# idonahum/photoVerse

Measured on AMD Instinct MI355X. Metric: denoising steps/sec at 512x512 bs=16, 50-step loop (2 UNet fwd + CFG + DPM-Solver++ step per step), higher is better.
Workload: dtype f16; 1 GPU; configs[1] shape timed over 96 steps instead of 50: SD-v1.5 UNet + PhotoVerse processors, 96-step loop, bs=16/GPU, 512x512 (64x64 latents), P=1, guidance 7.5, fp16; per_gpu_batch=16, global_batch=16, latent=64, parallelism=dp1 (batch-sharded, 1 all_gather), hip_graph=True, graph_branches=2

## Files before the change

### photoverse_amd/csrc/pv_rowgemm.hip

```cpp
#include "pv_common.h"
#include <stdlib.h>

namespace {

constexpr int RG_K = 320;
constexpr int RG_CHUNK = 160;
constexpr int RG_TILE = RG_CHUNK * 128;
constexpr int RG_SLOTS = 4;
constexpr int RG_SMEM = RG_SLOTS * RG_TILE;

struct pv_rowgemm_params_dev : pv_row_gemm_params {
    uint32_t w_bytes;
};

template <int N>
__device__ __forceinline__ void rg_wait_vmcnt() {
    static_assert(N >= 0 && N < 64, "vmcnt is a 6-bit field");
    asm volatile("s_waitcnt vmcnt(%0)" ::"n"(N) : "memory");
}

template <bool GEGLU>
__global__ __launch_bounds__(256, 2) void row_gemm_kernel(const pv_rowgemm_params_dev p) {
    constexpr int C = RG_K;
    constexpr int KK = C / 32;
    constexpr int KT = C / 64;
    constexpr int NFC = RG_CHUNK / 16;
    typedef unsigned uint4_t __attribute__((ext_vector_type(4)));
    typedef unsigned uint2_t __attribute__((ext_vector_type(2)));
    extern __shared__ __attribute__((aligned(16))) char smem[];

    const int lane = pv_lane_id(), wave = pv_wave_id();
    const int fr = lane & 15, g = lane >> 4;
    const int m0 = (int)blockIdx.x * 128;
    const int rows_here = min(128, p.M - m0);
    const int n_chunks = p.N / RG_CHUNK;
    const int NT = n_chunks * KT;

    const __amdgpu_buffer_rsrc_t rw = __builtin_amdgcn_make_buffer_rsrc(const_cast<void*>(p.w), 0, (int)p.w_bytes, 0x00020000);
    const __amdgpu_buffer_rsrc_t rx = __builtin_amdgcn_make_buffer_rsrc(const_cast<half_t*>(reinterpret_cast<const half_t*>(p.x)) + (size_t)m0 * p.ld_x, 0,
                                                                        rows_here * p.ld_x * 2, 0x00020000);
    const int ld_o = p.ld_out;
    const __amdgpu_buffer_rsrc_t ro = __builtin_amdgcn_make_buffer_rsrc(reinterpret_cast<half_t*>(p.out) + (size_t)m0 * ld_o, 0, rows_here * ld_o * 2, 0x00020000);

    const int lrow = lane >> 3;
    const unsigned w_lane_off = (unsigned)lrow * (unsigned)(C * 2) + (unsigned)(((lane & 7) ^ lrow) << 4);
    const unsigned piece_off = w_lane_off + (unsigned)(wave * 8) * (unsigned)(C * 2);
    auto issue_stage = [&](int t) {
        const int nc = t / KT, kt = t - nc * KT;
        char* dst = smem + (t & (RG_SLOTS - 1)) * RG_TILE;
        const int soff = nc * RG_CHUNK * (C * 2) + kt * 128;
#pragma unroll
        for (int i = 0; i < 5; ++i)
            __builtin_amdgcn_raw_ptr_buffer_load_lds(rw, PV_LDS_PTR(dst + (wave + 4 * i) * 1024), 16, (int)piece_off, soff + i * 32 * (C * 2), 0, 0);
    };
    auto wg_barrier = [&]() {
        asm volatile("s_waitcnt lgkmcnt(0)" ::: "memory");
        __builtin_amdgcn_s_barrier();
        asm volatile("" ::: "memory");
    };

    half8_t xf[KK][2];
    int mrow[2];
#pragma unroll
    for (int qi = 0; qi < 2; ++qi) {
        mrow[qi] = wave * 32 + qi * 16 + fr;
        const int off = mrow[qi] * p.ld_x * 2 + g * 16;
#pragma unroll
        for (int kk = 0; kk < KK; ++kk) xf[kk][qi] = __builtin_bit_cast(half8_t, __builtin_amdgcn_raw_buffer_load_b128(rx, off, kk * 64, 0));
    }
    issue_stage(0);
    issue_stage(1);
    if (p.x_norm) {
        const float* tab = p.x_norm + (size_t)(m0 / p.rows_per_image) * 2 * C + g * 8;
#pragma unroll
        for (int kk = 0; kk < KK; ++kk) {
            const float4_t s0 = *reinterpret_cast<const float4_t*>(tab + kk * 32), s1 = *reinterpret_cast<const float4_t*>(tab + kk * 32 + 4);
            const float4_t h0 = *reinterpret_cast<const float4_t*>(tab + C + kk * 32), h1 = *reinterpret_cast<const float4_t*>(tab + C + kk * 32 + 4);
#pragma unroll
            for (int qi = 0; qi < 2; ++qi)
#pragma unroll
                for (int j = 0; j < 8; ++j) xf[kk][qi][j] = (half_t)((float)xf[kk][qi][j] * (j < 4 ? s0[j & 3] : s1[j & 3]) + (j < 4 ? h0[j & 3] : h1[j & 3]));
        }
    }
    if (p.ln) {
        typedef _Float16 h2_t __attribute__((ext_vector_type(2)));
        const h2_t ones = h2_t{(half_t)1.0f, (half_t)1.0f};
#pragma unroll
        for (int qi = 0; qi < 2; ++qi) {
            float sum = 0.f;
#pragma unroll
            for (int kk = 0; kk < KK; ++kk)
#pragma unroll
                for (int j = 0; j < 4; ++j) sum = __builtin_amdgcn_fdot2(h2_t{xf[kk][qi][2 * j], xf[kk][qi][2 * j + 1]}, ones, sum, false);
            const float mean = pv_quad_sum(sum) * (1.0f / (float)C);
            const half_t mh = (half_t)mean;
            const h2_t nm = h2_t{(half_t)(-mh), (half_t)(-mh)};
            float sq = 0.f;
#pragma unroll
            for (int kk = 0; kk < KK; ++kk)
#pragma unroll
                for (int j = 0; j < 4; ++j) {
                    const h2_t d = h2_t{xf[kk][qi][2 * j], xf[kk][qi][2 * j + 1]} + nm;
                    sq = __builtin_amdgcn_fdot2(d, d, sq, false);
                }
            const float dm = mean - (float)mh;
            const float var = pv_quad_sum(sq) * (1.0f / (float)C) - dm * dm;
            const float rstd = rsqrtf(fmaxf(var, 0.f) + p.ln_eps);
            const float nmr = -mean * rstd;
#pragma unroll
            for (int kk = 0; kk < KK; ++kk)
#pragma unroll
                for (int j = 0; j < 8; ++j) xf[kk][qi][j] = (half_t)fmaf((float)xf[kk][qi][j], rstd, nmr);
        }
    }
    rg_wait_vmcnt<0>();

    const int ring_lane[2] = {fr * 128 + ((g ^ (fr & 7)) << 4), fr * 128 + (((4 + g) ^ (fr & 7)) << 4)};
    const int pcol = (g & 1) ? 16 + (g - 1) * 4 : g * 4;
    constexpr int OUT_PER_CHUNK = GEGLU ? RG_CHUNK / 2 : RG_CHUNK;
    constexpr int STORES = GEGLU ? 6 : 10;

    float4_t acc[NFC][2];
    for (int it = 0; it < n_chunks / 2; ++it) {
        const int t0 = it * (2 * KT);
#pragma unroll
        for (int j = 0; j < 2 * KT; ++j) {
            const int t = t0 + j;
            const int kt = j % KT;
            const int nc = 2 * it + j / KT;
            if ((j & 1) == 0) {
                const bool stores_since = (j == 6) || (j == 0 && it > 0);
                if (t >= 2) {
                    if (stores_since) rg_wait_vmcnt<STORES>(); else rg_wait_vmcnt<0>();
                }
                wg_barrier();
                if (t + 2 < NT) issue_stage(t + 2);
                if (t + 3 < NT) issue_stage(t + 3);
            }
            if (kt == 0) {
#pragma unroll
                for (int i = 0; i < NFC; ++i)
                    acc[i][0] = acc[i][1] = p.bias ? *reinterpret_cast<const float4_t*>(p.bias + nc * RG_CHUNK + i * 16 + g * 4) : float4_t{0.f, 0.f, 0.f, 0.f};
            }
            const char* slot = smem + (t & (RG_SLOTS - 1)) * RG_TILE;
#pragma unroll
            for (int ks = 0; ks < 2; ++ks) {
                const char* base = slot + ring_lane[ks];
#pragma unroll
                for (int i = 0; i < NFC; ++i) {
                    const half8_t a = *reinterpret_cast<const half8_t*>(base + i * 2048);
#pragma unroll
                    for (int qi = 0; qi < 2; ++qi) acc[i][qi] = __builtin_amdgcn_mfma_f32_16x16x32_f16(a, xf[2 * kt + ks][qi], acc[i][qi], 0, 0, 0);
                }
            }
            if (kt == KT - 1) {
                const int ocol0 = nc * OUT_PER_CHUNK;
#pragma unroll
                for (int qi = 0; qi < 2; ++qi) {
                    const int ooff = mrow[qi] * ld_o * 2 + ocol0 * 2;
                    unsigned pk[GEGLU ? NFC / 2 : NFC][2];
                    if (GEGLU) {
#pragma unroll
                        for (int q = 0; q < NFC / 2; ++q) {
                            const float4_t v = acc[2 * q][qi], gt = acc[2 * q + 1][qi];
                            pk[q][0] = __builtin_bit_cast(unsigned, half2_t{(half_t)(v[0] * pv_gelu_erf(gt[0])), (half_t)(v[1] * pv_gelu_erf(gt[1]))});
                            pk[q][1] = __builtin_bit_cast(unsigned, half2_t{(half_t)(v[2] * pv_gelu_erf(gt[2])), (half_t)(v[3] * pv_gelu_erf(gt[3]))});
                        }
                    } else {
#pragma unroll
                        for (int i = 0; i < NFC; ++i) {
                            const float4_t v = acc[i][qi];
                            pk[i][0] = __builtin_bit_cast(unsigned, half2_t{(half_t)v[0], (half_t)v[1]});
                            pk[i][1] = __builtin_bit_cast(unsigned, half2_t{(half_t)v[2], (half_t)v[3]});
                        }
                    }
                    constexpr int NOUT = GEGLU ? NFC / 2 : NFC;
#pragma unroll
                    for (int q = 0; q < NOUT / 2; ++q) {
                        const auto v0 = __builtin_amdgcn_permlane16_swap(pk[2 * q][0], pk[2 * q + 1][0], false, false);
                        const auto v1 = __builtin_amdgcn_permlane16_swap(pk[2 * q][1], pk[2 * q + 1][1], false, false);
                        const unsigned sa0 = v0[0], sb0 = v0[1], sa1 = v1[0], sb1 = v1[1];
                        __builtin_amdgcn_raw_buffer_store_b128(uint4_t{sa0, sa1, sb0, sb1}, ro, ooff + pcol * 2 + q * 64, 0, 0);
                        asm volatile("s_nop 1" ::: "memory");
                    }
                    if (NOUT & 1)
                        __builtin_amdgcn_raw_buffer_store_b64(uint2_t{pk[NOUT - 1][0], pk[NOUT - 1][1]}, ro, ooff + g * 8 + (NOUT - 1) * 32, 0, 0);
                }
                __builtin_amdgcn_sched_barrier(0);
            }
        }
    }
}

}

extern "C" int pv_row_gemm(const pv_row_gemm_params* pp, void* stream) {
    pv_rowgemm_params_dev p;
    static_cast<pv_row_gemm_params&>(p) = *pp;
    if (!p.x || !p.w || !p.out || p.M <= 0 || p.K != RG_K || p.N <= 0 || (p.N % (2 * RG_CHUNK)) || (p.ld_x % 8) || (p.ld_out % 8) || p.ld_x < RG_K ||
        p.ld_out < (p.geglu ? p.N / 2 : p.N) || (p.x_norm && (p.ln || p.rows_per_image <= 0 || (p.rows_per_image % 128) || (p.M % p.rows_per_image))))
        return (int)hipErrorInvalidValue;
    if ((size_t)p.N * RG_K * 2 >= (1ull << 31)) return (int)hipErrorInvalidValue;
    p.w_bytes = (uint32_t)p.N * RG_K * 2;
    static bool attr_set_dev[64][2] = {};
    int dev_id = 0;
    (void)hipGetDevice(&dev_id);
    bool& attr_set = attr_set_dev[dev_id & 63][p.geglu ? 1 : 0];
    auto kern = p.geglu ? row_gemm_kernel<true> : row_gemm_kernel<false>;
    if (!attr_set) {
        hipError_t e = hipFuncSetAttribute(reinterpret_cast<const void*>(kern), hipFuncAttributeMaxDynamicSharedMemorySize, RG_SMEM);
        if (e != hipSuccess) return (int)e;
        attr_set = true;
    }
    hipLaunchKernelGGL(kern, dim3((unsigned)((p.M + 127) / 128)), dim3(256), RG_SMEM, (hipStream_t)stream, p);
    return PV_CHECK_LAUNCH();
}
```

### photoverse_amd/csrc/pv_convbig.hip

```cpp
#include "pv_gemm_dev.h"

#ifndef PV_PATCH_ABLATE
#define PV_PATCH_ABLATE 0
#endif
#ifdef PV_CONVBIG_STAMPS
__device__ unsigned long long pv_convbig_stamps[3 * 8 * 8];
extern "C" int pv_convbig_read_stamps(unsigned long long* out) { return (int)hipMemcpyFromSymbol(out, HIP_SYMBOL(pv_convbig_stamps), sizeof(pv_convbig_stamps)); }
#define CB_DECL unsigned long long cb_acc[4] = {0, 0, 0, 0}, cb_t = __builtin_amdgcn_s_memtime(), cb_u, cb_r0 = __builtin_amdgcn_s_memrealtime(), cb_c0 = cb_t; int cb_n = 0;
#define CB_MARK(i) do { cb_u = __builtin_amdgcn_s_memtime(); cb_acc[i] += cb_u - cb_t; cb_t = cb_u; } while (0)
#define CB_COUNT() (++cb_n)
#define CB_DUMP() do { const int slot_ = blockIdx.x == 0 ? 0 : blockIdx.x == 50 ? 1 : blockIdx.x == 100 ? 2 : -1; \
        if (slot_ >= 0 && lane == 0) { unsigned long long* o_ = pv_convbig_stamps + (slot_ * 8 + wave) * 8; \
            o_[0] = cb_acc[0]; o_[1] = cb_acc[1]; o_[2] = cb_acc[2]; o_[3] = cb_acc[3]; o_[4] = cb_t - cb_c0; o_[5] = __builtin_amdgcn_s_memrealtime() - cb_r0; o_[6] = cb_n; } } while (0)
#else
#define CB_DECL
#define CB_MARK(i)
#define CB_COUNT()
#define CB_DUMP()
#endif

namespace {

constexpr int BK = 32;
constexpr int ROW_BYTES = BK * 2;
// ... 18 lines not shown
    static constexpr int SMEM_NORM_BYTES = SMEM_PATCH_BYTES + NORM_TABLE_BYTES;
};

__device__ __forceinline__ float epi_act(float x, int act) {
    if (act == PV_ACT_SILU) return pv_silu(x);
    if (act == PV_ACT_QUICK_GELU) return pv_quick_gelu(x);
    if (act == PV_ACT_LEAKY_RELU) return x > 0.f ? x : 0.01f * x;
    return x;
}

__device__ __forceinline__ int swz(int rq) { return (0x78 >> (2 * rq)) & 3; }

template <int N>
__device__ __forceinline__ void wait_vmcnt() {
    asm volatile("s_waitcnt vmcnt(%0)" ::"n"(N) : "memory");
}

__device__ __forceinline__ float row16_sum(float v) {
    v += __builtin_bit_cast(float, __builtin_amdgcn_update_dpp(0, __builtin_bit_cast(int, v), 0x128, 0xf, 0xf, false));
    v += __builtin_bit_cast(float, __builtin_amdgcn_update_dpp(0, __builtin_bit_cast(int, v), 0x124, 0xf, 0xf, false));
    v += __builtin_bit_cast(float, __builtin_amdgcn_update_dpp(0, __builtin_bit_cast(int, v), 0x122, 0xf, 0xf, false));
    v += __builtin_bit_cast(float, __builtin_amdgcn_update_dpp(0, __builtin_bit_cast(int, v), 0x121, 0xf, 0xf, false));
    return v;
}

template <int V>
struct IC { static constexpr int value = V; };

template <bool CS, bool UPS, int MI, int MODE, bool LN = false>
__global__ __launch_bounds__(512, 2) void big_tile_kernel(const pv_gemm_params_dev p, const int tiles_n, const int nblk) {
    constexpr int NF = MODE == 2 ? 4 : 5;
    constexpr bool PATCH = MODE >= 3, NORMA = MODE >= 5;
    constexpr bool IS_CONV = MODE == 0 || PATCH;
    constexpr int LOG2W = (MODE == 3 || MODE == 5) ? 6 : 5, PW = 1 << LOG2W, PR = 256 >> LOG2W, PS = PW + 2, NPIX = (PR + 2) * PS;
    constexpr int TAPS = IS_CONV ? 9 : 1;
    using Cfg = BigCfg<MI, NF>;
    static_assert(!PATCH || (MI == 8 && !UPS && !LN), "the patch modes are the plain 256-row conv");
    static_assert(NPIX <= Cfg::PATCH_PIECES * 16, "the patch fits its 32 pieces");
    constexpr int BM = Cfg::BM, BN = Cfg::BN, AP = Cfg::AP, BP = Cfg::BP, B_PIECES = Cfg::B_PIECES, A_BYTES = Cfg::A_BYTES, STAGE_BYTES = Cfg::STAGE_BYTES;
    constexpr int P_HI = AP + BP, P_LO = AP + Cfg::BP_LO;
    static_assert(!UPS || MODE == 0, "the upsampling gather belongs to the conv");
    static_assert(!LN || (MODE != 0 && !CS), "the LayerNorm fold exists for the Linear modes (their outputs feed attention / a Linear: no column statistics)");
    extern __shared__ __attribute__((aligned(16))) char smem[];
    const int lane = pv_lane_id();
    const int wave = pv_wave_id();
    const int bid = pv_xcd_remap((int)blockIdx.x, nblk);
    const int tile_m = bid / tiles_n, tile_n = bid - tile_m * tiles_n;
    const int m0 = tile_m * BM, n0 = tile_n * BN;
    const int cin = p.c0 + p.c1;
    const int K = TAPS * cin;
    const int nk64 = K / 64;
    const int nk_per = (nk64 + (int)gridDim.y - 1) / (int)gridDim.y;
    const int kb = (int)blockIdx.y * nk_per;
    const int ns = 2 * max(0, min(nk64, kb + nk_per) - kb);

    constexpr unsigned OOB = 0x80000000u;
    const int hw_out = p.hout * p.wout;
    const int prow = lane >> 2;
    float4_t acc[NF][MI];
#pragma unroll
    for (int ni = 0; ni < NF; ++ni)
#pragma unroll
        for (int mi = 0; mi < MI; ++mi) acc[ni][mi] = float4_t{0.f, 0.f, 0.f, 0.f};

    const int wm = wave >> 2, wn = wave & 3;
    const int fr = lane & 15, fq = lane >> 4;
    const int arow = wm * (MI * 16) + fr;
    const int brow = wn * (NF * 16) + fr;
    const int frag_off = fr * ROW_BYTES + ((fq ^ swz((fr >> 2) & 3)) << 4);

    half8_t wb[NF], xa[MI];
    float ln_s1[LN ? MI : 1], ln_s2[LN ? MI : 1];
#pragma unroll
    for (int mi = 0; mi < (LN ? MI : 1); ++mi) ln_s1[mi] = ln_s2[mi] = 0.f;
    auto seg_barrier = [&]() {
        __builtin_amdgcn_sched_barrier(0);
        __builtin_amdgcn_s_barrier();
        asm volatile("" ::: "memory");
        __builtin_amdgcn_sched_barrier(0);
    };
    if constexpr (!PATCH) {
        const int lane_cc2 = ((lane & 3) ^ swz((lane >> 4) & 3)) * 16;
        const __amdgpu_buffer_rsrc_t ra0 = __builtin_amdgcn_make_buffer_rsrc(const_cast<void*>(p.a0), 0, (int)p.a0_bytes, 0x00020000);
        const __amdgpu_buffer_rsrc_t ra1 = __builtin_amdgcn_make_buffer_rsrc(const_cast<void*>(p.a1 ? p.a1 : p.a0), 0, (int)p.a1_bytes, 0x00020000);
        const __amdgpu_buffer_rsrc_t rw = __builtin_amdgcn_make_buffer_rsrc(const_cast<void*>(p.w), 0, (int)p.w_bytes, 0x00020000);
        unsigned a_off0[AP], a_off1[AP], a_mask[AP];
#pragma unroll
        for (int i = 0; i < AP; ++i) {
            const int m = m0 + (wave + i * NW) * 16 + prow;
            const bool ok = m < p.M;
            if (MODE != 0) {
                a_off0[i] = ok ? (unsigned)m * (unsigned)(p.lda0 * 2) + lane_cc2 : OOB;
                a_off1[i] = a_mask[i] = 0;
                continue;
            }
            const int b = m / hw_out;
            const int rem = m - b * hw_out;
            const int y = rem / p.wout, x = rem - y * p.wout;
            const int hl = UPS ? 2 * p.hin : p.hin, wl = UPS ? 2 * p.win : p.win;
            unsigned mask = 0;
#pragma unroll
            for (int t = 0; t < 9; ++t) {
                const int iy = y + t / 3 - 1, ix = x + t % 3 - 1;
                mask |= (ok && iy >= 0 && iy < hl && ix >= 0 && ix < wl) ? 1u << t : 0u;
            }
            if (UPS) mask |= (unsigned)(y & 1) << 9 | (unsigned)(x & 1) << 10;
            a_mask[i] = mask;
            const unsigned pix = UPS ? (unsigned)((b * p.hin + (y >> 1)) * p.win + (x >> 1)) : (unsigned)((b * p.hin + y) * p.win + x);
            a_off0[i] = pix * (unsigned)(p.lda0 * 2) + lane_cc2;
            a_off1[i] = pix * (unsigned)(p.lda1 * 2) + lane_cc2;
        }
        unsigned w_off[BP];
#pragma unroll
        for (int i = 0; i < BP; ++i) w_off[i] = (unsigned)(n0 + min(wave + i * NW, B_PIECES - 1) * 16 + prow) * (unsigned)(K * 2) + lane_cc2;
        const bool b_full = wave + (BP - 1) * NW < B_PIECES;

        struct KPos { int s, chunk, tap, ky, kx; };
        auto kpos_of = [&](int s) {
            const int g = kb + (s >> 1), chunk = g / TAPS, tap = g - chunk * TAPS, ky = TAPS == 9 ? tap / 3 : 1;
            return KPos{s, chunk, tap, ky, TAPS == 9 ? tap - ky * 3 : 1};
        };
        auto kpos_next = [&](KPos& k) {
            if (k.s & 1) {
                if (TAPS == 9) {
                    ++k.tap; ++k.kx;
                    if (k.kx == 3) { k.kx = 0; ++k.ky; }
                    if (k.tap == 9) { k.tap = 0; k.ky = 0; ++k.chunk; }
                } else {
                    ++k.chunk;
                }
            }
            ++k.s;
        };
        auto issue = [&](const KPos& k, auto j0c, auto j1c) {
            constexpr int J0 = decltype(j0c)::value, J1 = decltype(j1c)::value;
            char* sa = smem + (k.s & (NBUF - 1)) * STAGE_BYTES;
            char* sb = sa + A_BYTES;
            const int c = k.chunk * 64 + (k.s & 1) * BK;
            const bool first = c < p.c0;
            const __amdgpu_buffer_rsrc_t ra = first ? ra0 : ra1;
            const int ld2 = (first ? p.lda0 : p.lda1) * 2;
            const int sc2 = (first ? c : c - p.c0) * 2;
            const int tap_delta = ((k.ky - 1) * p.win + (k.kx - 1)) * ld2 + sc2;
            const int oy_even = (k.ky == 0 ? -p.win : 0) * ld2, oy_odd = (k.ky == 2 ? p.win : 0) * ld2;
            const int ox_even = (k.kx == 0 ? -1 : 0) * ld2, ox_odd = (k.kx == 2 ? 1 : 0) * ld2;
            const unsigned wk2 = (unsigned)(k.tap * cin + c) * 2u;
            const unsigned tap_bit = 1u << k.tap;
#pragma unroll
            for (int j = J0; j < J1; ++j) {
                if (j < AP && MODE != 0) {
                    const unsigned off = a_off0[j] == OOB ? OOB : a_off0[j] + (unsigned)(c * 2);
                    __builtin_amdgcn_raw_ptr_buffer_load_lds(ra0, PV_LDS_PTR(sa + (wave + j * NW) * 16 * ROW_BYTES), 16, (int)off, 0, 0, 0);
                } else if (j < AP) {
                    unsigned off = first ? a_off0[j] : a_off1[j];
                    if (UPS) off += (unsigned)(((a_mask[j] >> 9) & 1u ? oy_odd : oy_even) + ((a_mask[j] >> 10) & 1u ? ox_odd : ox_even) + sc2);
                    else off += (unsigned)tap_delta;
                    off = (a_mask[j] & tap_bit) ? off : OOB;
                    __builtin_amdgcn_raw_ptr_buffer_load_lds(ra, PV_LDS_PTR(sa + (wave + j * NW) * 16 * ROW_BYTES), 16, (int)off, 0, 0, 0);
                } else if (j - AP < BP - 1 || b_full) {
                    __builtin_amdgcn_raw_ptr_buffer_load_lds(rw, PV_LDS_PTR(sb + (wave + (j - AP) * NW) * 16 * ROW_BYTES), 16, (int)(w_off[j - AP] + wk2), 0, 0, 0);
                }
            }
        };

        auto read_frags = [&](int s) {
            const char* sa = smem + (s & (NBUF - 1)) * STAGE_BYTES + wm * (MI * 16) * ROW_BYTES + frag_off;
            const char* sb = smem + (s & (NBUF - 1)) * STAGE_BYTES + A_BYTES + wn * (NF * 16) * ROW_BYTES + frag_off;
#pragma unroll
            for (int ni = 0; ni < NF; ++ni) wb[ni] = *reinterpret_cast<const half8_t*>(sb + ni * 16 * ROW_BYTES);
#pragma unroll
            for (int mi = 0; mi < MI; ++mi) xa[mi] = *reinterpret_cast<const half8_t*>(sa + mi * 16 * ROW_BYTES);
        };
        {
            const int pre = min(ns, 3);
            for (int s = 0; s < pre; ++s) issue(kpos_of(s), IC<0>{}, IC<AP + BP>{});
            if (pre == 3) { if (wm == 0) wait_vmcnt<2 * P_HI>(); else wait_vmcnt<2 * P_LO>(); }
            else wait_vmcnt<0>();
        }
        seg_barrier();
        if (wm == 1) seg_barrier();

        KPos kn = kpos_of(3);
        CB_DECL
        for (int s = 0; s < ns; ++s) {
            CB_COUNT();
            read_frags(s);
            if (s + 3 < ns) issue(kn, IC<0>{}, IC<AP + BP>{});
            kpos_next(kn);
            if (wm == 1) {
                if (s + 3 < ns) wait_vmcnt<2 * P_LO>(); else wait_vmcnt<0>();
            }
            asm volatile("s_waitcnt lgkmcnt(0)" ::: "memory");
            CB_MARK(0);
            seg_barrier();
            CB_MARK(1);
#pragma unroll
            for (int mi = 0; mi < MI; ++mi) {
#pragma unroll
                for (int ni = 0; ni < NF; ++ni)
                    acc[ni][mi] = __builtin_amdgcn_mfma_f32_16x16x32_f16(wb[ni], xa[mi], acc[ni][mi], 0, 0, 0);
                if constexpr (LN) {
                    const half2_t one2 = half2_t{(half_t)1.0f, (half_t)1.0f};
#pragma unroll
                    for (int j = 0; j < 4; ++j) {
                        const half2_t x2 = half2_t{xa[mi][2 * j], xa[mi][2 * j + 1]};
                        ln_s1[mi] = __builtin_amdgcn_fdot2(x2, one2, ln_s1[mi], false);
                        ln_s2[mi] = __builtin_amdgcn_fdot2(x2, x2, ln_s2[mi], false);
                    }
                }
            }
            if (wm == 0) {
                if (s + 3 < ns) wait_vmcnt<2 * P_HI>(); else wait_vmcnt<0>();
            }
            CB_MARK(2);
            seg_barrier();
            CB_MARK(3);
        }
        CB_DUMP();
        if (wm == 0) seg_barrier();

    } else {
        constexpr int B_BYTES = Cfg::B_BYTES, PATCH_BYTES = Cfg::PATCH_BYTES;
        constexpr int PB_HI = BP, PB_LO = Cfg::BP_LO;
        char* const s_patch = smem + NBUF * B_BYTES;
        const __amdgpu_buffer_rsrc_t ra0 = __builtin_amdgcn_make_buffer_rsrc(const_cast<void*>(p.a0), 0, (int)p.a0_bytes, 0x00020000);
        const __amdgpu_buffer_rsrc_t ra1 = __builtin_amdgcn_make_buffer_rsrc(const_cast<void*>(p.a1 ? p.a1 : p.a0), 0, (int)p.a1_bytes, 0x00020000);
        const __amdgpu_buffer_rsrc_t rw = __builtin_amdgcn_make_buffer_rsrc(const_cast<void*>(p.w), 0, (int)p.w_bytes, 0x00020000);
        const int nchunk = cin / BK;
        const int nst = 9 * nchunk;
        const int img = m0 / hw_out, y0 = (m0 - img * hw_out) >> LOG2W;
        unsigned ppix[4];
#pragma unroll
        for (int i = 0; i < 4; ++i) {
            const int pp = 16 * (wave + 8 * i) + prow;
            const int py = pp / PS, px = pp - py * PS;
            const int iy = y0 - 1 + py, ix = px - 1;
            const bool ok = pp < NPIX && iy >= 0 && iy < p.hin && ix >= 0 && ix < PW;
            ppix[i] = ok ? (unsigned)((img * p.hin + iy) * PW + ix) : OOB;
        }
        const unsigned patch_cc = (unsigned)(((lane & 3) ^ (((lane >> 4) & 1) << 1)) * 16);
        const int lane_cc2 = ((lane & 3) ^ swz((lane >> 4) & 3)) * 16;
        const unsigned w_off = (unsigned)(n0 + wave * 16 + prow) * (unsigned)(K * 2) + lane_cc2;
        const int w_piece_step = NW * 16 * K * 2;
        const bool b_full = wave + (BP - 1) * NW < B_PIECES;
        auto issue_w = [&](int s, int chunk, int tap) {
            char* sb = smem + (s & (NBUF - 1)) * B_BYTES;
            const int wk2 = (tap * cin + chunk * BK) * 2;
#pragma unroll
            for (int j = 0; j < BP; ++j)
                if (j < BP - 1 || b_full)
                    __builtin_amdgcn_raw_ptr_buffer_load_lds(rw, PV_LDS_PTR(sb + (wave + j * NW) * 16 * ROW_BYTES), 16, (int)w_off, wk2 + j * w_piece_step, 0, 0);
        };
        int ld2_0 = p.lda0 * 2, ld2_1 = p.lda1 * 2, c0s = p.c0;
        asm volatile("" : "+s"(ld2_0), "+s"(ld2_1), "+s"(c0s));
        auto issue_patch = [&](int chunk, int i) {
            const int c = chunk * BK;
            const bool first = c < c0s;
            const unsigned ld2 = (unsigned)(first ? ld2_0 : ld2_1), sc2 = (unsigned)(first ? c : c - c0s) * 2u;
            const unsigned px = ppix[0];
            ppix[0] = ppix[1]; ppix[1] = ppix[2]; ppix[2] = ppix[3]; ppix[3] = px;
            const unsigned off = px == OOB ? OOB : px * ld2 + sc2 + patch_cc;
            char* dst = s_patch + (chunk & 1) * PATCH_BYTES + (wave + 8 * i) * 16 * ROW_BYTES;
            const __amdgpu_buffer_rsrc_t ra = first ? ra0 : ra1;
            __builtin_amdgcn_raw_ptr_buffer_load_lds(ra, PV_LDS_PTR(dst), 16, (int)off, 0, 0, 0);
        };
        const int lane_pp = (wm * (128 >> LOG2W)) * PS + fr;
        constexpr int NROW = (MI * 16) >> LOG2W, FPR = PW / 16;
        unsigned a_row[NROW];
        auto frag_addrs = [&](int chunk, int tapshift) {
            const int base = lane_pp + tapshift;
            const unsigned buf = (unsigned)(NBUF * B_BYTES + (chunk & 1) * PATCH_BYTES);
#pragma unroll
            for (int r = 0; r < NROW; ++r) {
                const int pp = base + r * PS;
                a_row[r] = buf + (unsigned)pp * ROW_BYTES + (unsigned)((fq ^ ((pp >> 1) & 2)) << 4);
            }
        };
        auto read_frags_p = [&](int s) {
            const char* sb = smem + (s & (NBUF - 1)) * B_BYTES + wn * (NF * 16) * ROW_BYTES + frag_off;
#pragma unroll
            for (int ni = 0; ni < NF; ++ni) wb[ni] = *reinterpret_cast<const half8_t*>(sb + ni * 16 * ROW_BYTES);
#pragma unroll
            for (int mi = 0; mi < MI; ++mi) xa[mi] = *reinterpret_cast<const half8_t*>(smem + a_row[mi / FPR] + (mi % FPR) * 16 * ROW_BYTES);
        };
        float* const s_tab = reinterpret_cast<float*>(smem + Cfg::SMEM_PATCH_BYTES);
        const int lane_dc8 = ((lane & 3) ^ (((lane >> 4) & 1) << 1)) * 8;
        auto norm_piece = [&](int chunk, int i) {
            const unsigned px = ppix[0];
            ppix[0] = ppix[1]; ppix[1] = ppix[2]; ppix[2] = ppix[3]; ppix[3] = px;
            char* at = s_patch + (chunk & 1) * PATCH_BYTES + (wave + 8 * i) * 16 * ROW_BYTES + lane * 16;
            const half8_t v = *reinterpret_cast<const half8_t*>(at);
            const float* sc = s_tab + chunk * BK + lane_dc8;
            const float4_t s0 = *reinterpret_cast<const float4_t*>(sc), s1 = *reinterpret_cast<const float4_t*>(sc + 4);
            const float4_t h0 = *reinterpret_cast<const float4_t*>(sc + cin), h1 = *reinterpret_cast<const float4_t*>(sc + cin + 4);
            half8_t o;
#pragma unroll
            for (int j = 0; j < 8; ++j) {
                float f = (float)v[j] * (j < 4 ? s0[j & 3] : s1[j & 3]) + (j < 4 ? h0[j & 3] : h1[j & 3]);
                if (p.a_norm_act == PV_ACT_SILU) f = f * __builtin_amdgcn_rcpf(1.0f + __builtin_amdgcn_exp2f(-1.4426950408889634f * f));
                o[j] = (half_t)f;
            }
            if (px != OOB) *reinterpret_cast<half8_t*>(at) = o;
        };
        if constexpr (NORMA) {
            const float* tab = p.a_norm + (size_t)img * 2 * cin;
            for (int i = (int)threadIdx.x; i < 2 * cin; i += NW * 64) s_tab[i] = tab[i];
        }
#pragma unroll
        for (int i = 0; i < 4; ++i) issue_patch(0, i);
        for (int s = 0; s < 3; ++s) issue_w(s, 0, s);
        if (wm == 0) wait_vmcnt<2 * PB_HI>(); else wait_vmcnt<2 * PB_LO>();
        if constexpr (NORMA) {
            __syncthreads();
#pragma unroll
            for (int i = 0; i < 4; ++i) norm_piece(0, i);
            asm volatile("s_waitcnt lgkmcnt(0)" ::: "memory");
        }
        frag_addrs(0, 0);
        seg_barrier();
        if (wm == 1) seg_barrier();

        int chunk = 0, tap = 0, kx = 0, tapshift = 0;
        int c3 = 0, t3 = 3;
        CB_DECL
        for (int s = 0; s < nst; ++s) {
            CB_COUNT();
            read_frags_p(s);
#if PV_PATCH_ABLATE == 2
            const int e_now = 0;
#else
            const int e_now = (tap < 4 && chunk + 1 < nchunk) ? 1 : 0;
#endif
            if (s + 3 < nst) issue_w(s + 3, c3, t3);
            if (e_now) issue_patch(chunk + 1, tap);
            if (++t3 == 9) { t3 = 0; ++c3; }
            if (wm == 1) {
                if (s + 3 < nst) wait_vmcnt<2 * PB_LO>(); else wait_vmcnt<0>();
            }
            asm volatile("s_waitcnt lgkmcnt(0)" ::: "memory");
            CB_MARK(0);
            seg_barrier();
            CB_MARK(1);
            ++tap; ++kx; ++tapshift;
            if (kx == 3) { kx = 0; tapshift += PS - 3; }
            if (tap == 9) { tap = 0; tapshift = 0; ++chunk; }
#if PV_PATCH_ABLATE != 1
            frag_addrs(chunk, tapshift);
#endif
            if constexpr (NORMA) {
                if (tap >= 5 && chunk + 1 < nchunk) norm_piece(chunk + 1, tap - 5);
            }
#pragma unroll
            for (int mi = 0; mi < MI; ++mi)
#pragma unroll
                for (int ni = 0; ni < NF; ++ni)
                    acc[ni][mi] = __builtin_amdgcn_mfma_f32_16x16x32_f16(wb[ni], xa[mi], acc[ni][mi], 0, 0, 0);
#pragma unroll
            for (int r = 0; r < NROW; ++r) asm volatile("" : "+v"(a_row[r]));
#if PV_PATCH_ABLATE != 4
#pragma unroll
            for (int g = 0; g < MI; ++g) {
                __builtin_amdgcn_sched_group_barrier(0x008, NF, 0);
                __builtin_amdgcn_sched_group_barrier(0x006, 4, 0);
            }
#endif
            if (wm == 0) {
                if (s + 3 < nst) wait_vmcnt<2 * PB_HI>(); else wait_vmcnt<0>();
            }
            CB_MARK(2);
            seg_barrier();
            CB_MARK(3);
        }
        CB_DUMP();
        if (wm == 0) seg_barrier();
    }

    const int nbase = n0 + wn * (NF * 16) + fq * 4;
    if (gridDim.y > 1) {
        float* slab = p.splitk_ws + (size_t)blockIdx.y * p.M * p.N;
#pragma unroll
        for (int mi = 0; mi < MI; ++mi) {
            const int m = m0 + arow + mi * 16;
            if (m >= p.M) continue;
#pragma unroll
            for (int ni = 0; ni < NF; ++ni) *reinterpret_cast<float4_t*>(slab + (size_t)m * p.N + nbase + ni * 16) = acc[ni][mi];
        }
        return;
    }
    if constexpr (LN) {
#pragma unroll
        for (int mi = 0; mi < MI; ++mi) {
            const float a = pv_quad_sum(ln_s1[mi]) / (float)K, q2 = pv_quad_sum(ln_s2[mi]) / (float)K;
            ln_s1[mi] = a;
            ln_s2[mi] = rsqrtf(fmaxf(q2 - a * a, 0.f) + p.ln_eps);
        }
    }
    auto ln_fold = [&](float4_t v, const float4_t rs, int mi) {
        if constexpr (LN) {
#pragma unroll
            for (int r = 0; r < 4; ++r) v[r] = ln_s2[mi] * (v[r] - ln_s1[mi] * rs[r]);
        }
        return v;
    };
    if constexpr (MODE == 2) {
        float4_t bv[2], bg[2];
#pragma unroll
        for (int q = 0; q < 2; ++q) {
            bv[q] = p.bias ? *reinterpret_cast<const float4_t*>(p.bias + nbase + (2 * q) * 16) : float4_t{0.f, 0.f, 0.f, 0.f};
            bg[q] = p.bias ? *reinterpret_cast<const float4_t*>(p.bias + nbase + (2 * q + 1) * 16) : float4_t{0.f, 0.f, 0.f, 0.f};
        }
        float4_t rv[2], rg[2];
#pragma unroll
        for (int q = 0; q < 2; ++q) {
            rv[q] = LN ? *reinterpret_cast<const float4_t*>(p.ln_rowsum + nbase + (2 * q) * 16) : float4_t{0.f, 0.f, 0.f, 0.f};
            rg[q] = LN ? *reinterpret_cast<const float4_t*>(p.ln_rowsum + nbase + (2 * q + 1) * 16) : float4_t{0.f, 0.f, 0.f, 0.f};
        }
#pragma unroll
        for (int mi = 0; mi < MI; ++mi) {
            const int m = m0 + arow + mi * 16;
            if (m >= p.M) continue;
            unsigned pk[2][2];
#pragma unroll
            for (int q = 0; q < 2; ++q) {
                const float4_t v = ln_fold(acc[2 * q][mi], rv[q], mi) + bv[q], g = ln_fold(acc[2 * q + 1][mi], rg[q], mi) + bg[q];
                pk[q][0] = __builtin_bit_cast(unsigned, half2_t{(half_t)(v[0] * pv_gelu_erf(g[0])), (half_t)(v[1] * pv_gelu_erf(g[1]))});
                pk[q][1] = __builtin_bit_cast(unsigned, half2_t{(half_t)(v[2] * pv_gelu_erf(g[2])), (half_t)(v[3] * pv_gelu_erf(g[3]))});
            }
            half_t* orow = reinterpret_cast<half_t*>(p.out) + (size_t)m * p.ldc + (n0 >> 1) + wn * (NF * 8);
            const auto r0 = __builtin_amdgcn_permlane16_swap(pk[0][0], pk[1][0], false, false);
            const auto r1 = __builtin_amdgcn_permlane16_swap(pk[0][1], pk[1][1], false, false);
            const unsigned a0 = r0[0], b0 = r0[1], a1 = r1[0], b1 = r1[1];
            const int col = (fq & 1) ? 16 + (fq - 1) * 4 : fq * 4;
            typedef unsigned uint4_t __attribute__((ext_vector_type(4)));
            *reinterpret_cast<uint4_t*>(orow + col) = uint4_t{a0, a1, b0, b1};
        }
        return;
    }
    float* s_bias = reinterpret_cast<float*>(smem);
    float* s_rs = s_bias + BN;
    float* s_radd = s_rs + BN;
    static_assert((2 + 2 * (MI / 4)) * BN * 4 <= BigCfg<MI, NF>::SMEM_BYTES, "the epilogue staging must fit the ring");
    if constexpr (NF == 5) {
        const int tid = (int)threadIdx.x;
        for (int i = tid; i < BN; i += NW * 64) {
            s_bias[i] = p.bias ? p.bias[n0 + i] : 0.f;
            if (LN) s_rs[i] = p.ln_rowsum[n0 + i];
        }
        if (IS_CONV && p.rowadd) {
            for (int i = tid; i < 2 * (MI / 4) * BN; i += NW * 64) {
                const int blk = i / BN, c = i - blk * BN;
                const int img = min(m0 + blk * 64, p.M - 1) / hw_out;
                s_radd[i] = p.rowadd[(size_t)img * p.rowadd_ld + n0 + c];
            }
        }
        __syncthreads();
    }
    const int ncol = wn * (NF * 16) + fq * 4;
    const bool want_cs = CS && p.colstats != nullptr;
    typedef unsigned uint4_t __attribute__((ext_vector_type(4)));
    typedef unsigned uint2_t __attribute__((ext_vector_type(2)));
    auto block = [&](int hb) {
        const int mb0 = m0 + wm * (MI * 16) + hb * 64;
        const bool one_image = IS_CONV && p.rowadd && (mb0 / hw_out) == (min(mb0 + 63, p.M - 1) / hw_out);
        const float* s_ra = s_radd + (wm * (MI / 4) + hb) * BN + ncol;
        constexpr int RBUF = CS ? 1 : 2;
        half4_t res[RBUF][NF];
        auto fetch_res = [&](int q) {
            const int mm = min(m0 + arow + (hb * 4 + q) * 16, p.M - 1);
#pragma unroll
            for (int t = 0; t < NF; ++t)
                res[q % RBUF][t] = *reinterpret_cast<const half4_t*>(reinterpret_cast<const half_t*>(p.residual) + (size_t)mm * p.ldr + nbase + t * 16);
        };
        if (RBUF == 2 && p.residual) fetch_res(0);
        float4_t cs[NF], cq[NF];
#pragma unroll
        for (int t = 0; t < NF; ++t) cs[t] = cq[t] = float4_t{0.f, 0.f, 0.f, 0.f};
#pragma unroll
        for (int q = 0; q < 4; ++q) {
            const int mi = hb * 4 + q;
            if (p.residual && (RBUF == 1 || q + 1 < 4)) fetch_res(RBUF == 1 ? q : q + 1);
            const int m = m0 + arow + mi * 16;
            if (m >= p.M) continue;
            asm volatile("" ::: "memory");
            const float* radd = (p.rowadd && !one_image) ? p.rowadd + (size_t)(m / hw_out) * p.rowadd_ld + nbase : nullptr;
            half_t* orow = reinterpret_cast<half_t*>(p.out) + (size_t)m * p.ldc + n0 + wn * (NF * 16);
            auto value = [&](int t, unsigned (&pk)[2]) {
                float4_t v = acc[t][mi];
                if constexpr (LN) v = ln_fold(v, *reinterpret_cast<const float4_t*>(s_rs + ncol + t * 16), mi);
                v += *reinterpret_cast<const float4_t*>(s_bias + ncol + t * 16);
                if (IS_CONV && one_image) v += *reinterpret_cast<const float4_t*>(s_ra + t * 16);
                else if (radd) v += *reinterpret_cast<const float4_t*>(radd + t * 16);
                if (p.act) {
#pragma unroll
                    for (int r = 0; r < 4; ++r) v[r] = epi_act(v[r], p.act);
                }
                if (p.residual) {
#pragma unroll
                    for (int r = 0; r < 4; ++r) v[r] += (float)res[q % RBUF][t][r];
                }
                const half4_t hv = half4_t{(half_t)v[0], (half_t)v[1], (half_t)v[2], (half_t)v[3]};
                pk[0] = __builtin_bit_cast(unsigned, half2_t{hv[0], hv[1]});
                pk[1] = __builtin_bit_cast(unsigned, half2_t{hv[2], hv[3]});
                if (want_cs) {
#pragma unroll
                    for (int r = 0; r < 4; ++r) {
                        const float f = (float)hv[r];
                        cs[t][r] += f;
                        cq[t][r] += f * f;
                    }
                }
            };
#pragma unroll
            for (int t = 0; t + 1 < NF; t += 2) {
                unsigned pa[2], pb[2];
                value(t, pa);
                value(t + 1, pb);
                const auto r0 = __builtin_amdgcn_permlane16_swap(pa[0], pb[0], false, false);
                const auto r1 = __builtin_amdgcn_permlane16_swap(pa[1], pb[1], false, false);
                const unsigned a0 = r0[0], b0 = r0[1], a1 = r1[0], b1 = r1[1];
                const int col = (fq & 1) ? (t + 1) * 16 + (fq - 1) * 4 : t * 16 + fq * 4;
                *reinterpret_cast<uint4_t*>(orow + col) = uint4_t{a0, a1, b0, b1};
                asm volatile("" ::: "memory");
            }
            if constexpr (NF & 1) {
                unsigned pa[2];
                value(NF - 1, pa);
                *reinterpret_cast<uint2_t*>(orow + (NF - 1) * 16 + fq * 4) = uint2_t{pa[0], pa[1]};
            }
        }
        if (want_cs && mb0 < p.M) {
#pragma unroll
            for (int t = 0; t < NF; ++t)
#pragma unroll
                for (int r = 0; r < 4; ++r) {
                    cs[t][r] = row16_sum(cs[t][r]);
                    cq[t][r] = row16_sum(cq[t][r]);
                }
            if (fr == 0) {
                float* dst = p.colstats + ((size_t)(m0 / 64 + wm * (MI / 4) + hb) * 2) * p.N + nbase;
#pragma unroll
                for (int t = 0; t < NF; ++t) {
                    *reinterpret_cast<float4_t*>(dst + t * 16) = cs[t];
                    *reinterpret_cast<float4_t*>(dst + p.N + t * 16) = cq[t];
                }
            }
        }
    };
    if constexpr (NF == 5) {
#pragma unroll
        for (int hb = 0; hb < MI / 4; ++hb) block(hb);
    }
}

template <bool CS, bool UPS, int MI, int MODE, bool LN = false>
int launch_big(const pv_gemm_params_dev& p, hipStream_t stream) {
    using Cfg = BigCfg<MI, MODE == 2 ? 4 : 5>;
    constexpr int BM = Cfg::BM, BN = Cfg::BN, SMEM_BYTES = MODE >= 5 ? Cfg::SMEM_NORM_BYTES : MODE >= 3 ? Cfg::SMEM_PATCH_BYTES : Cfg::SMEM_BYTES;
    if (pv_gemm_probe) {
        snprintf(pv_gemm_probe->name, sizeof(pv_gemm_probe->name), "big_tile_kernel<%s, %s, %d, %d, %s>", CS ? "true" : "false", UPS ? "true" : "false", MI, MODE,
                 LN ? "true" : "false");
        pv_gemm_probe->wgs = (long)((p.M + BM - 1) / BM) * (p.N / BN) * ((p.splitk > 1 && p.splitk_ws) ? p.splitk : 1);
        return 0;
    }
    static bool attr_set_dev[64] = {};
    int dev_id = 0;
    (void)hipGetDevice(&dev_id);
    bool& attr_set = attr_set_dev[dev_id & 63];
    auto kern = big_tile_kernel<CS, UPS, MI, MODE, LN>;
    if (!attr_set) {
        hipError_t e = hipFuncSetAttribute(reinterpret_cast<const void*>(kern), hipFuncAttributeMaxDynamicSharedMemorySize, SMEM_BYTES);
        if (e != hipSuccess) return (int)e;
        attr_set = true;
    }
    const int tiles_m = (p.M + BM - 1) / BM, tiles_n = p.N / BN;
    const int splits = (p.splitk > 1 && p.splitk_ws) ? p.splitk : 1;
    hipLaunchKernelGGL(kern, dim3(tiles_m * tiles_n, splits), dim3(NW * 64), SMEM_BYTES, stream, p, tiles_n, tiles_m * tiles_n);
    if (splits > 1) return pv_gemm_splitk_reduce_launch(p, splits, stream);
    return PV_CHECK_LAUNCH();
}

}

int pv_conv_big_launch(const pv_gemm_params_dev& p, hipStream_t stream) {
    const char* env = getenv("PV_CONV_BIG");
    const int min_tiles = p.big_tile_min ? p.big_tile_min : (env ? atoi(env) : 256);
    if (min_tiles <= 0) return p.a_norm ? -2 : -1;
    const int splits = (p.splitk > 1 && p.splitk_ws) ? p.splitk : 1;
    const int cin = p.c0 + p.c1;
    if (p.taps == 1) {
        const char* genv = getenv("PV_GEMM_BIG");
        if (genv && atoi(genv) == 0) return -1;
        const int bn = p.geglu ? 256 : 320;
        if (p.c1 || splits > 1 || p.out_f32 || cin < 640 || (p.N % bn) || (p.geglu && p.colstats)) return -1;
        if ((long)((p.M + 255) / 256) * (p.N / bn) < min_tiles) {
            static const int b128 = getenv("PV_GEMM_BIG128") ? atoi(getenv("PV_GEMM_BIG128")) : 0;
            if (b128 && !p.geglu && !p.ln_rowsum && cin >= (b128 > 1 ? b128 : 1280) && (long)((p.M + 127) / 128) * (p.N / bn) >= (min_tiles > 256 ? min_tiles : 256))
                return p.colstats ? launch_big<true, false, 4, 1>(p, stream) : launch_big<false, false, 4, 1>(p, stream);
            return -1;
        }
        if (p.ln_rowsum) {
            if (p.colstats) return -1;
            return p.geglu ? launch_big<false, false, 8, 2, true>(p, stream) : launch_big<false, false, 8, 1, true>(p, stream);
        }
        if (p.geglu) return launch_big<false, false, 8, 2>(p, stream);
        return p.colstats ? launch_big<true, false, 8, 1>(p, stream) : launch_big<false, false, 8, 1>(p, stream);
    }
    constexpr int BN = 320;
    const int up = p.upsample ? 2 : 1;
    const bool shape_ok = p.taps == 9 && p.stride == 1 && p.pad == 1 && p.hin * up == p.hout && p.win * up == p.wout && (p.N % BN) == 0 &&
                          !p.geglu;
    if (!shape_ok) return -1;
    if (splits == 1 && p.out_f32) return -1;
    if (splits > 1 && (9 * cin / 64) / splits < 8) return -1;
    const long tiles256 = (long)((p.M + 255) / 256) * (p.N / BN) * splits;
    if (tiles256 < min_tiles) return -1;
    const bool cs = p.colstats && splits == 1;
    const char* penv = getenv("PV_CONV_PATCH");
    const int pmode = penv ? atoi(penv) : 64;
    if (pmode != 0 && !p.upsample && splits == 1 && (p.wout == 64 || (p.wout == 32 && pmode != 64)) && ((p.hout * p.wout) % 256) == 0 && (p.M % 256) == 0 &&
        (p.c0 % 32) == 0 && (cin % 32) == 0) {
        if (p.a_norm) {
            if (2 * cin * 4 > BigCfg<8, 5>::NORM_TABLE_BYTES) return -2;
            if (p.wout == 64) return cs ? launch_big<true, false, 8, 5>(p, stream) : launch_big<false, false, 8, 5>(p, stream);
            return cs ? launch_big<true, false, 8, 6>(p, stream) : launch_big<false, false, 8, 6>(p, stream);
        }
        if (p.wout == 64) return cs ? launch_big<true, false, 8, 3>(p, stream) : launch_big<false, false, 8, 3>(p, stream);
        return cs ? launch_big<true, false, 8, 4>(p, stream) : launch_big<false, false, 8, 4>(p, stream);
    }
    if (p.a_norm) return -2;
    if (p.upsample) return cs ? launch_big<true, true, 8, 0>(p, stream) : launch_big<false, true, 8, 0>(p, stream);
    return cs ? launch_big<true, false, 8, 0>(p, stream) : launch_big<false, false, 8, 0>(p, stream);
}
```

Before: 32.18 denoising steps/s (bs=16 per GPU, summed over GPUs).

## Share weight ring across two 128-row halves in 512-thread row GEMM blocks

Each block now covers 256 rows with 512 threads, so two groups of four waves share one LDS weight ring and each weight tile is fetched once per 256 rows instead of once per 128. The ring grows to six slots and is filled in stage pairs, with an optional lag between the two halves. Bias is staged in LDS, and large N is split across several launches to fit the LDS budget. LDS fragment loads are issued ahead of the MFMAs and interleaved with sched_group_barrier. The cost is occupancy: one 512-thread block per CU instead of two 256-thread blocks, plus extra launches when N is large.

```diff
diff --git a/photoverse_amd/csrc/pv_rowgemm.hip b/photoverse_amd/csrc/pv_rowgemm.hip
--- a/photoverse_amd/csrc/pv_rowgemm.hip
+++ b/photoverse_amd/csrc/pv_rowgemm.hip
@@ -6,8 +6,26 @@
 constexpr int RG_K = 320;
 constexpr int RG_CHUNK = 160;
 constexpr int RG_TILE = RG_CHUNK * 128;
-constexpr int RG_SLOTS = 4;
+constexpr int RG_ROWS = 256;
+#ifndef PV_RG_SLOTS
+#define PV_RG_SLOTS 6
+#endif
+#ifndef PV_RG_LAG_PLAIN
+#define PV_RG_LAG_PLAIN 1
+#endif
+#ifndef PV_RG_LAG_GEGLU
+#define PV_RG_LAG_GEGLU 0
+#endif
+#ifndef PV_RG_PF
+#define PV_RG_PF 6
+#endif
+constexpr int RG_PF = PV_RG_PF;
+constexpr int RG_SLOTS = PV_RG_SLOTS;
+template <bool GEGLU> constexpr int rg_lag() { return GEGLU ? PV_RG_LAG_GEGLU : PV_RG_LAG_PLAIN; }
 constexpr int RG_SMEM = RG_SLOTS * RG_TILE;
+constexpr int RG_LDS_MAX = 160 * 1024;
+constexpr int RG_NMAX = (RG_LDS_MAX - RG_SMEM) / 4 / (2 * RG_CHUNK) * (2 * RG_CHUNK);
+static_assert(RG_SLOTS % 2 == 0 && RG_NMAX >= 2 * RG_CHUNK, "the ring holds whole stage pairs and leaves room for a bias in the CU's LDS");
 
 struct pv_rowgemm_params_dev : pv_row_gemm_params {
     uint32_t w_bytes;
@@ -20,21 +38,24 @@
 }
 
 template <bool GEGLU>
-__global__ __launch_bounds__(256, 2) void row_gemm_kernel(const pv_rowgemm_params_dev p) {
+__global__ __launch_bounds__(512, 1) void row_gemm_kernel(const pv_rowgemm_params_dev p) {
     constexpr int C = RG_K;
     constexpr int KK = C / 32;
     constexpr int KT = C / 64;
     constexpr int NFC = RG_CHUNK / 16;
+    constexpr int RG_LAG = rg_lag<GEGLU>();
+    static_assert(RG_LAG >= 0 && RG_LAG <= RG_SLOTS / 2 - 2, "pair G + 1 is written over pair G + 1 - RG_SLOTS / 2 in interval G: its last reader must be done");
     typedef unsigned uint4_t __attribute__((ext_vector_type(4)));
     typedef unsigned uint2_t __attribute__((ext_vector_type(2)));
     extern __shared__ __attribute__((aligned(16))) char smem[];
 
     const int lane = pv_lane_id(), wave = pv_wave_id();
     const int fr = lane & 15, g = lane >> 4;
-    const int m0 = (int)blockIdx.x * 128;
-    const int rows_here = min(128, p.M - m0);
+    const int half = wave >> 2;
+    const int m0 = (int)blockIdx.x * RG_ROWS;
+    const int rows_here = min(RG_ROWS, p.M - m0);
     const int n_chunks = p.N / RG_CHUNK;
-    const int NT = n_chunks * KT;
+    const int NP = n_chunks * KT / 2;
 
     const __amdgpu_buffer_rsrc_t rw = __builtin_amdgcn_make_buffer_rsrc(const_cast<void*>(p.w), 0, (int)p.w_bytes, 0x00020000);
     const __amdgpu_buffer_rsrc_t rx = __builtin_amdgcn_make_buffer_rsrc(const_cast<half_t*>(reinterpret_cast<const half_t*>(p.x)) + (size_t)m0 * p.ld_x, 0,
@@ -45,13 +66,23 @@
     const int lrow = lane >> 3;
     const unsigned w_lane_off = (unsigned)lrow * (unsigned)(C * 2) + (unsigned)(((lane & 7) ^ lrow) << 4);
     const unsigned piece_off = w_lane_off + (unsigned)(wave * 8) * (unsigned)(C * 2);
-    auto issue_stage = [&](int t) {
+    const int piece5 = 16 + (wave & 3);
+    const unsigned piece5_off = w_lane_off + (unsigned)(piece5 * 8) * (unsigned)(C * 2);
+    auto issue_pair = [&](int P) {
+#pragma unroll
+        for (int s = 0; s < 2; ++s) {
+            const int t = 2 * P + s;
+            const int nc = t / KT, kt = t - nc * KT;
+            char* dst = smem + (t % RG_SLOTS) * RG_TILE;
+            const int soff = nc * RG_CHUNK * (C * 2) + kt * 128;
+#pragma unroll
+            for (int i = 0; i < 2; ++i)
+                __builtin_amdgcn_raw_ptr_buffer_load_lds(rw, PV_LDS_PTR(dst + (wave + 8 * i) * 1024), 16, (int)piece_off, soff + i * 64 * (C * 2), 0, 0);
+        }
+        const int t = 2 * P + half;
         const int nc = t / KT, kt = t - nc * KT;
-        char* dst = smem + (t & (RG_SLOTS - 1)) * RG_TILE;
-        const int soff = nc * RG_CHUNK * (C * 2) + kt * 128;
-#pragma unroll
-        for (int i = 0; i < 5; ++i)
-            __builtin_amdgcn_raw_ptr_buffer_load_lds(rw, PV_LDS_PTR(dst + (wave + 4 * i) * 1024), 16, (int)piece_off, soff + i * 32 * (C * 2), 0, 0);
+        __builtin_amdgcn_raw_ptr_buffer_load_lds(rw, PV_LDS_PTR(smem + (t % RG_SLOTS) * RG_TILE + piece5 * 1024), 16, (int)piece5_off,
+                                                 nc * RG_CHUNK * (C * 2) + kt * 128, 0, 0);
     };
     auto wg_barrier = [&]() {
         asm volatile("s_waitcnt lgkmcnt(0)" ::: "memory");
@@ -68,10 +99,13 @@
 #pragma unroll
         for (int kk = 0; kk < KK; ++kk) xf[kk][qi] = __builtin_bit_cast(half8_t, __builtin_amdgcn_raw_buffer_load_b128(rx, off, kk * 64, 0));
     }
-    issue_stage(0);
-    issue_stage(1);
+    issue_pair(0);
+    const float* bias_l = reinterpret_cast<const float*>(smem + RG_SMEM);
+    for (int i = (int)threadIdx.x; i < p.N / 4; i += 512)
+        reinterpret_cast<float4_t*>(smem + RG_SMEM)[i] = p.bias ? reinterpret_cast<const float4_t*>(p.bias)[i] : float4_t{0.f, 0.f, 0.f, 0.f};
     if (p.x_norm) {
-        const float* tab = p.x_norm + (size_t)(m0 / p.rows_per_image) * 2 * C + g * 8;
+        const int mh = m0 + 128 * half < p.M ? m0 + 128 * half : m0;
+        const float* tab = p.x_norm + (size_t)(mh / p.rows_per_image) * 2 * C + g * 8;
 #pragma unroll
         for (int kk = 0; kk < KK; ++kk) {
             const float4_t s0 = *reinterpret_cast<const float4_t*>(tab + kk * 32), s1 = *reinterpret_cast<const float4_t*>(tab + kk * 32 + 4);
@@ -121,6 +155,12 @@
     constexpr int STORES = GEGLU ? 6 : 10;
 
     float4_t acc[NFC][2];
+    if (half)
+        for (int G = 0; G < RG_LAG; ++G) {
+            rg_wait_vmcnt<0>();
+            wg_barrier();
+            if (G + 1 < NP) issue_pair(G + 1);
+        }
     for (int it = 0; it < n_chunks / 2; ++it) {
         const int t0 = it * (2 * KT);
 #pragma unroll
@@ -130,29 +170,36 @@
             const int nc = 2 * it + j / KT;
             if ((j & 1) == 0) {
                 const bool stores_since = (j == 6) || (j == 0 && it > 0);
-                if (t >= 2) {
-                    if (stores_since) rg_wait_vmcnt<STORES>(); else rg_wait_vmcnt<0>();
-                }
+                const int G = (t >> 1) + half * RG_LAG;
+                if (stores_since) rg_wait_vmcnt<STORES>(); else rg_wait_vmcnt<0>();
                 wg_barrier();
-                if (t + 2 < NT) issue_stage(t + 2);
-                if (t + 3 < NT) issue_stage(t + 3);
+                if (G + 1 < NP) issue_pair(G + 1);
             }
             if (kt == 0) {
 #pragma unroll
+                for (int i = 0; i < NFC; ++i) acc[i][0] = acc[i][1] = *reinterpret_cast<const float4_t*>(bias_l + nc * RG_CHUNK + i * 16 + g * 4);
+            }
+            const char* slot = smem + (t % RG_SLOTS) * RG_TILE;
+            __builtin_amdgcn_sched_barrier(0);
+            half8_t a[2 * NFC];
+#pragma unroll
+            for (int ks = 0; ks < 2; ++ks)
+#pragma unroll
+                for (int i = 0; i < NFC; ++i) a[ks * NFC + i] = *reinterpret_cast<const half8_t*>(slot + ring_lane[ks] + i * 2048);
+#pragma unroll
+            for (int ks = 0; ks < 2; ++ks)
+#pragma unroll
                 for (int i = 0; i < NFC; ++i)
-                    acc[i][0] = acc[i][1] = p.bias ? *reinterpret_cast<const float4_t*>(p.bias + nc * RG_CHUNK + i * 16 + g * 4) : float4_t{0.f, 0.f, 0.f, 0.f};
-            }
-            const char* slot = smem + (t & (RG_SLOTS - 1)) * RG_TILE;
-#pragma unroll
-            for (int ks = 0; ks < 2; ++ks) {
-                const char* base = slot + ring_lane[ks];
-#pragma unroll
-                for (int i = 0; i < NFC; ++i) {
-                    const half8_t a = *reinterpret_cast<const half8_t*>(base + i * 2048);
-#pragma unroll
-                    for (int qi = 0; qi < 2; ++qi) acc[i][qi] = __builtin_amdgcn_mfma_f32_16x16x32_f16(a, xf[2 * kt + ks][qi], acc[i][qi], 0, 0, 0);
-                }
-            }
+#pragma unroll
+                    for (int qi = 0; qi < 2; ++qi) acc[i][qi] = __builtin_amdgcn_mfma_f32_16x16x32_f16(a[ks * NFC + i], xf[2 * kt + ks][qi], acc[i][qi], 0, 0, 0);
+            __builtin_amdgcn_sched_group_barrier(0x100, RG_PF, 0);
+#pragma unroll
+            for (int n = 0; n < 2 * NFC - RG_PF; ++n) {
+                __builtin_amdgcn_sched_group_barrier(0x008, 2, 0);
+                __builtin_amdgcn_sched_group_barrier(0x100, 1, 0);
+            }
+            __builtin_amdgcn_sched_group_barrier(0x008, 2 * RG_PF, 0);
+            if (kt != KT - 1) __builtin_amdgcn_sched_barrier(0);
             if (kt == KT - 1) {
                 const int ocol0 = nc * OUT_PER_CHUNK;
 #pragma unroll
@@ -190,6 +237,8 @@
             }
         }
     }
+    if (!half)
+        for (int G = 0; G < RG_LAG; ++G) wg_barrier();
 }
 
 }
@@ -201,17 +250,23 @@
         p.ld_out < (p.geglu ? p.N / 2 : p.N) || (p.x_norm && (p.ln || p.rows_per_image <= 0 || (p.rows_per_image % 128) || (p.M % p.rows_per_image))))
         return (int)hipErrorInvalidValue;
     if ((size_t)p.N * RG_K * 2 >= (1ull << 31)) return (int)hipErrorInvalidValue;
-    p.w_bytes = (uint32_t)p.N * RG_K * 2;
     static bool attr_set_dev[64][2] = {};
     int dev_id = 0;
     (void)hipGetDevice(&dev_id);
     bool& attr_set = attr_set_dev[dev_id & 63][p.geglu ? 1 : 0];
     auto kern = p.geglu ? row_gemm_kernel<true> : row_gemm_kernel<false>;
     if (!attr_set) {
-        hipError_t e = hipFuncSetAttribute(reinterpret_cast<const void*>(kern), hipFuncAttributeMaxDynamicSharedMemorySize, RG_SMEM);
+        hipError_t e = hipFuncSetAttribute(reinterpret_cast<const void*>(kern), hipFuncAttributeMaxDynamicSharedMemorySize, RG_LDS_MAX);
         if (e != hipSuccess) return (int)e;
         attr_set = true;
     }
-    hipLaunchKernelGGL(kern, dim3((unsigned)((p.M + 127) / 128)), dim3(256), RG_SMEM, (hipStream_t)stream, p);
+    for (int n0 = 0; n0 < pp->N; n0 += RG_NMAX) {
+        p.N = pp->N - n0 < RG_NMAX ? pp->N - n0 : RG_NMAX;
+        p.w = static_cast<const char*>(pp->w) + (size_t)n0 * RG_K * 2;
+        p.bias = pp->bias ? pp->bias + n0 : nullptr;
+        p.out = static_cast<char*>(pp->out) + (size_t)(p.geglu ? n0 / 2 : n0) * 2;
+        p.w_bytes = (uint32_t)p.N * RG_K * 2;
+        hipLaunchKernelGGL(kern, dim3((unsigned)((p.M + RG_ROWS - 1) / RG_ROWS)), dim3(512), RG_SMEM + p.N * 4, (hipStream_t)stream, p);
+    }
     return PV_CHECK_LAUNCH();
 }
```

Result: no change. 32.43 denoising steps/s (bs=16 per GPU, summed over GPUs), median of 6 (+0.8%).

## Split fused norm+SiLU of conv patches into fetch/apply interleaved with MFMAs

Applied to the files above, without the earlier changes.

The GroupNorm+SiLU pass over the staged input patch, which used to run as a whole piece only in taps 5-8, is now split into a half-piece LDS fetch issued before the barrier and an apply step run every tap. Scheduling barriers interleave the transcendental ops and the LDS store with the MFMA block. The goal is to hide the normalisation ALU and LDS latency behind matrix work and to spread it evenly across taps. The cost is more register pressure, branchless masking for out-of-bounds pixels, and tricky timing dependencies on which patch pieces each tap reads.

```diff
diff --git a/photoverse_amd/csrc/pv_convbig.hip b/photoverse_amd/csrc/pv_convbig.hip
--- a/photoverse_amd/csrc/pv_convbig.hip
+++ b/photoverse_amd/csrc/pv_convbig.hip
@@ -344,6 +344,34 @@
             }
             if (px != OOB) *reinterpret_cast<half8_t*>(at) = o;
         };
+        half4_t n_v = {};
+        float4_t n_s = {}, n_h = {};
+        unsigned n_at = 0, n_keep = 0;
+        const bool n_silu = p.a_norm_act == PV_ACT_SILU;
+        unsigned n_ok = 0;
+#pragma unroll
+        for (int i = 0; i < 4; ++i) n_ok |= ppix[i] != OOB ? 1u << i : 0u;
+        auto norm_fetch = [&](bool act, int chunk, int i, int half) {
+            const int pc = act ? wave + 8 * i : Cfg::PATCH_PIECES - 1, tc = act ? chunk : 0;
+            n_at = (unsigned)(NBUF * B_BYTES + (tc & 1) * PATCH_BYTES + pc * 16 * ROW_BYTES + half * 8) + (unsigned)lane * 16u;
+            n_keep = act ? 0u - ((n_ok >> i) & 1u) : 0u;
+            n_v = *reinterpret_cast<const half4_t*>(smem + n_at);
+            const float* sc = s_tab + tc * BK + half * 4 + lane_dc8;
+            n_s = *reinterpret_cast<const float4_t*>(sc);
+            n_h = *reinterpret_cast<const float4_t*>(sc + cin);
+        };
+        auto norm_apply = [&]() {
+            half4_t o;
+#pragma unroll
+            for (int j = 0; j < 4; ++j) {
+                const float f = (float)n_v[j] * n_s[j] + n_h[j];
+                const float g = f * __builtin_amdgcn_rcpf(1.0f + __builtin_amdgcn_exp2f(-1.4426950408889634f * f));
+                o[j] = (half_t)(n_silu ? g : f);
+            }
+            typedef unsigned uint2_t __attribute__((ext_vector_type(2)));
+            const uint2_t ob = __builtin_bit_cast(uint2_t, o);
+            *reinterpret_cast<uint2_t*>(smem + n_at) = uint2_t{ob[0] & n_keep, ob[1] & n_keep};
+        };
         if constexpr (NORMA) {
             const float* tab = p.a_norm + (size_t)img * 2 * cin;
             for (int i = (int)threadIdx.x; i < 2 * cin; i += NW * 64) s_tab[i] = tab[i];
@@ -375,6 +403,12 @@
 #endif
             if (s + 3 < nst) issue_w(s + 3, c3, t3);
             if (e_now) issue_patch(chunk + 1, tap);
+            if constexpr (NORMA) {
+                static_assert(PR * PS <= 16 * (2 * NW + NW / 2), "tap 0 reads nothing of the pieces 2 that waves 4-7 normalise in tap 8");
+                const int early = tap < 2;
+                const int act = early ? (int)(chunk > 0) : ((int)(tap > 2) & (int)(chunk + 1 < nchunk));
+                norm_fetch(act != 0, chunk + 1 - early, early ? 3 : (max(tap, 3) - 3) >> 1, early ? tap : (tap - 3) & 1);
+            }
             if (++t3 == 9) { t3 = 0; ++c3; }
             if (wm == 1) {
                 if (s + 3 < nst) wait_vmcnt<2 * PB_LO>(); else wait_vmcnt<0>();
@@ -383,27 +417,38 @@
             CB_MARK(0);
             seg_barrier();
             CB_MARK(1);
-            ++tap; ++kx; ++tapshift;
-            if (kx == 3) { kx = 0; tapshift += PS - 3; }
-            if (tap == 9) { tap = 0; tapshift = 0; ++chunk; }
+            auto mfma_block = [&]() {
+                ++tap; ++kx; ++tapshift;
+                if (kx == 3) { kx = 0; tapshift += PS - 3; }
+                if (tap == 9) { tap = 0; tapshift = 0; ++chunk; }
 #if PV_PATCH_ABLATE != 1
-            frag_addrs(chunk, tapshift);
+                frag_addrs(chunk, tapshift);
 #endif
-            if constexpr (NORMA) {
-                if (tap >= 5 && chunk + 1 < nchunk) norm_piece(chunk + 1, tap - 5);
-            }
-#pragma unroll
-            for (int mi = 0; mi < MI; ++mi)
-#pragma unroll
-                for (int ni = 0; ni < NF; ++ni)
-                    acc[ni][mi] = __builtin_amdgcn_mfma_f32_16x16x32_f16(wb[ni], xa[mi], acc[ni][mi], 0, 0, 0);
-#pragma unroll
-            for (int r = 0; r < NROW; ++r) asm volatile("" : "+v"(a_row[r]));
+#pragma unroll
+                for (int mi = 0; mi < MI; ++mi)
+#pragma unroll
+                    for (int ni = 0; ni < NF; ++ni)
+                        acc[ni][mi] = __builtin_amdgcn_mfma_f32_16x16x32_f16(wb[ni], xa[mi], acc[ni][mi], 0, 0, 0);
+#pragma unroll
+                for (int r = 0; r < NROW; ++r) asm volatile("" : "+v"(a_row[r]));
+            };
+            if constexpr (NORMA) norm_apply();
+            mfma_block();
 #if PV_PATCH_ABLATE != 4
 #pragma unroll
             for (int g = 0; g < MI; ++g) {
                 __builtin_amdgcn_sched_group_barrier(0x008, NF, 0);
-                __builtin_amdgcn_sched_group_barrier(0x006, 4, 0);
+                if constexpr (!NORMA) {
+                    __builtin_amdgcn_sched_group_barrier(0x006, 4, 0);
+                } else if (g < 4) {
+                    __builtin_amdgcn_sched_group_barrier(0x006, 4, 0);
+                    __builtin_amdgcn_sched_group_barrier(0x400, 1, 0);
+                    __builtin_amdgcn_sched_group_barrier(0x006, 4, 0);
+                    __builtin_amdgcn_sched_group_barrier(0x400, 1, 0);
+                    __builtin_amdgcn_sched_group_barrier(0x006, 2, 0);
+                } else {
+                    __builtin_amdgcn_sched_group_barrier(0x006, 10, 0);
+                }
             }
 #endif
             if (wm == 0) {
```

Result: no change. 32.92 denoising steps/s (bs=16 per GPU, summed over GPUs) before, 32.91 denoising steps/s (bs=16 per GPU, summed over GPUs) after (median of 2 runs) (-0.0%).
